# DiTEC-project/gnn-pressure-estimation

Hardware: AMD Instinct MI355X
Metric: train snapshots/sec (higher is better)
Workload: dtype f32; 1 GPU; gatres_small (15 blocks, nc=32), C-Town-sized WDN (388 nodes, 860 directed edges), batch_size=32 per GPU, fp32, full training step (device mask 0.95 -> fwd -> masked MSE -> bwd -> Adam), fused per-snapshot kernel (8 CUs per snapshot, row-window tables), hipGraph replay (20 steps per graph launch); global_batch=32, parallelism=dp1, plan_relabelled=False, row_window=92, dropped_steps=0, captured_graphs=25

## Files before the change

gnn-pressure-estimation_amd/csrc/gatres_layout.h:

```cpp
#pragma once
#include "gatres_common.h"

static inline __host__ __device__ int64_t r4(int64_t v) { return (v + 3) & ~(int64_t)3; }
#define GATRES_UREC_WORDS 128

struct Layout {
  int nb, nc;
  int64_t N, Eg;
  int64_t p_lin0_w, p_lin0_b, p_block0, p_block_stride, p_lin1_w, p_lin1_b, P;
  int64_t c1_as, c1_ad, c1_b, c1_W, c2_as, c2_ad, c2_b, c2_W;
  int64_t s_xin, s_h1, s_as1, s_ad1, s_al1, s_o1, s_h2, s_as2, s_ad2, s_al2, s_stride, saved_total;
  int64_t sc_y2, sc_ev, sc_xa, sc_xb, sc_gpa, sc_gpb, sc_gy2, sc_ge, sc_gad, sc_gas, sc_gh, sc_go1, sc_wt,
      sc_ge2, sc_gad2, sc_gas2, sc_gh2, sc_slabs, sc_loss_part, scratch_total;
  int64_t sc_px, sc_pmask, sc_pout, sc_pgout, sc_pgx;
  int64_t sc_wb;
  int64_t sc_xch, xch_stride;
  int64_t sc_urec;
  int64_t sc_keep, keep_stride, k_gh1, k_gh2, k_gas1, k_gad1, k_gas2, k_gad2;
  int split_max;
  int64_t sc_flags, flag_words, col_words, sc_part_slabs;
  int num_slabs;
  int slab_rows;
  int64_t slab_stride;
};
// ... 32 lines not shown
  int64_t o = 0;
  X.f1h = o; o += mn * 2 * nc;
  X.f1a = o; o += mn * 2;
  X.f2h = o; o += mn * nc;
  X.f2a = o; o += mn;
  X.f3 = o;  o += mn * nc;
  X.b1 = o;  o += mn * nc;
  X.b2y = o; o += mn * nc;
  X.b2e = o; o += me;
  X.b3o = o; o += mn * 2 * nc;
  X.b3e = o; o += me * 2;
  X.hb = o;  o += 6 * 8;
  X.total = (o + 15) & ~(int64_t)15;
  return X;
}

static inline bool make_layout(const gatres_model_t* m, int64_t N, int64_t Eg, int num_segments, int fused_nodes,
                               int fused_edges, Layout* L) {
  if (!m || m->num_blocks < 0 || N <= 0 || Eg < 0) return false;
  const int nc = m->nc, nb = m->num_blocks;
  if (nc < 4 || nc > 128 || !gatres_is_pow2(nc)) return false;
  L->nb = nb; L->nc = nc; L->N = N; L->Eg = Eg;
  const int64_t w = 2LL * nc * nc;
  L->p_lin0_w = 0; L->p_lin0_b = nc; L->p_block0 = 2LL * nc;
  L->c1_as = 0; L->c1_ad = 2LL * nc; L->c1_b = 4LL * nc; L->c1_W = 6LL * nc;
  L->c2_as = 6LL * nc + w; L->c2_ad = L->c2_as + nc; L->c2_b = L->c2_ad + nc; L->c2_W = L->c2_b + nc;
  L->p_block_stride = 9LL * nc + 2 * w;
  L->p_lin1_w = L->p_block0 + nb * L->p_block_stride;
  L->p_lin1_b = L->p_lin1_w + nc;
  L->P = L->p_lin1_b + 1;
// ... 62 lines not shown
    L->xch_stride = 2 * X.total;
    o += (int64_t)num_segments * L->xch_stride;
  }
  L->sc_urec = o;
  if (L->xch_stride > 0) o += (int64_t)((num_segments + 7) / 8) * 8 * 8 * GATRES_UREC_WORDS;
  L->sc_wb = o;    o += r4((int64_t)nb * 4 * nc * nc);
  L->sc_px = o;    o += r4(N);
  L->sc_pmask = o; o += r4((N + 3) / 4);
  L->sc_pout = o;  o += r4(N);
  L->sc_pgout = o; o += r4(N);
  L->sc_pgx = o;   o += r4(N);
  L->scratch_total = o;
  return true;
}

static inline int fused_nodes_of(const gatres_graph_t* g) {
  return (g && g->num_segments > 0 && g->seg_ptr && g->max_segment_nodes > 0 && g->max_segment_nodes <= 4096)
             ? g->max_segment_nodes : 0;
}
static inline bool make_layout_g(const gatres_model_t* m, const gatres_graph_t* g, Layout* L) {
  return g && make_layout(m, g->num_nodes, g->num_edges_gat, g->num_segments, fused_nodes_of(g),
                          g->max_segment_edges_gat, L);
}

constexpr int FUSED_STATUS_FAULT = 0, FUSED_STATUS_FAULT_COUNT = 1, FUSED_STATUS_FAULT_TICKETS = 2,
              FUSED_STATUS_DROPPED_STEPS = 3, FUSED_STATUS_SNAPSHOT = 8;
static inline int64_t fused_status_offset(const Layout& L) { return L.sc_flags + L.flag_words - 32; }
static inline unsigned* fused_status(float* scratch, const Layout& L) {
  return reinterpret_cast<unsigned*>(scratch + fused_status_offset(L));
}
// ... 28 lines not shown
```

gnn-pressure-estimation_amd/csrc/k_autoclip.hip:

```cpp
#include "gatres_common.h"
#include "k_autoclip.h"
#include "k_mask.h"
#include "k_update.h"

namespace {

constexpr int AC_NORM_MAX_BLOCKS = 256;
constexpr int AC_UPDATE_MAX_BLOCKS = 512;

__global__ __launch_bounds__(256) void autoclip_norm_kernel(const float* __restrict__ g, long long count, float grad_scale,
                                                            double* __restrict__ partials, unsigned long long* __restrict__ ctl,
                                                            const unsigned long long* __restrict__ step_counter, int drop_nan) {
  __shared__ double lds4[4];
  double s = 0.0;
  for (long long i = (long long)blockIdx.x * 256 + threadIdx.x; i < count; i += (long long)gridDim.x * 256) {
    const double x = (double)(g[i] * grad_scale);
    s += x * x;
  }
  s = ac_block_sum(s, lds4);
  if (threadIdx.x == 0) {
    partials[blockIdx.x] = s;
    if (blockIdx.x == 0) ac_snapshot(ctl, step_counter, drop_nan && g[0] != g[0]);
  }
}
// ... 94 lines not shown
  const long long gstride = (long long)a.update_blocks * 256;
  for (long long i = (long long)blockIdx.x * 256 + tid; i < t; i += gstride) B[i] = sorted_at(i);
  for (long long idx = (long long)blockIdx.x * 256 + tid; idx < a.u.count; idx += gstride) {
    const float pv = a.u.p[idx];
    float gv = a.u.g[idx] * a.u.grad_scale;
    gv = gv * coef;
    gv = gv + (float)wd * pv;
    float mv = a.u.m[idx];
    mv = mv + (float)(1.0 - b1) * (gv - mv);
    const float vv = (float)b2 * a.u.v[idx] + (float)(1.0 - b2) * gv * gv;
    const float denom = sqrtf(vv) / s_bc2_sqrt + (float)eps;
    const float pn = pv + (-s_step_size * mv) / denom;
    a.u.p[idx] = pn;
    a.u.m[idx] = mv;
    a.u.v[idx] = vv;
    if (a.u.wt) {
      const long long nc = a.u.nc, per = 2LL * nc * nc, stride = 9LL * nc + 2 * per, off = idx - 2LL * nc;
      if (off >= 0 && off < (long long)a.u.nb * stride) {
        const long long b = off / stride, o = off % stride;
        if (o >= 6LL * nc && o < 6LL * nc + per) {
          const long long e = o - 6LL * nc, row = e / nc, col = e % nc;
          a.u.wt[b * 2 * per + col * 2 * nc + row] = pn;
        } else if (o >= 9LL * nc + per) {
          const long long e = o - 9LL * nc - per, row = e / (2 * nc), col = e % (2 * nc);
          a.u.wt[b * 2 * per + per + col * nc + row] = pn;
        }
      }
    }
  }
}

bool ac_valid(const gatres_autoclip_t* ac) {
  return ac && ac->log && ac->sorted[0] && ac->sorted[1] && ac->sorted[0] != ac->sorted[1] && ac->ctl && ac->partials &&
         ac->norm_out && ac->clip_out && ac->coef_out && ac->capacity > 0 && ac->partials_cap > 0 &&
         ac->percentile >= 0.0 && ac->percentile <= 100.0;
}

}

extern "C" int32_t gatres_autoclip_partials(int64_t count) {
  return count <= 0 ? 0 : (int32_t)((count + 255) / 256);
}

// ... 47 lines not shown
```

gnn-pressure-estimation_amd/csrc/k_fused_host.hip:

```cpp
#include <atomic>
#include <vector>
#include "k_fused_dev.h"
#include "k_mask.h"
#include "k_autoclip.h"
#include "k_update.h"

namespace {

static unsigned long long* g_stamps = nullptr;
static int g_stamp_cap = 0;

struct SlabSumArgs {
  const float* slabs;
  int num_slabs, num_loss;
  long long stride;
  float* grads;
  const float* loss_part;
  float* loss;
  int do_adam, use_snap, reduce_blocks;
  unsigned* status;
  double* ac_partials;
  unsigned long long* ac_ctl;
};

// ... 64 lines not shown
    if constexpr (NORM) {
      const double x = (double)(acc * a.grad_scale);
      sq = fault ? 0.0 : x * x;
    }
    if (r.do_adam && !fault) {
      float gv = acc * a.grad_scale;
      gv = gv + (float)wd * pv;
      float mv = mv0;
      mv = mv + (float)(1.0 - b1) * (gv - mv);
      const float vv = (float)b2 * vv0 + (float)(1.0 - b2) * gv * gv;
      const float denom = sqrtf(vv) / s_bc2_sqrt + (float)eps;
      const float pn = pv + (-s_step_size * mv) / denom;
      a.p[idx] = pn;
      a.m[idx] = mv;
      a.v[idx] = vv;
      if (a.wt) {
        const long long per = 2LL * a.nc * a.nc, stride = 9LL * a.nc + 2 * per, off = idx - 2LL * a.nc;
        if (off >= 0 && off < (long long)a.nb * stride) {
          const long long b = off / stride, o = off % stride;
          if (o >= 6LL * a.nc && o < 6LL * a.nc + per) {
            const long long e = o - 6LL * a.nc, row = e / a.nc, col = e % a.nc;
            a.wt[b * 2 * per + col * 2 * a.nc + row] = pn;
          } else if (o >= 9LL * a.nc + per) {
            const long long e = o - 9LL * a.nc - per, row = e / (2 * a.nc), col = e % (2 * a.nc);
            a.wt[b * 2 * per + per + col * a.nc + row] = pn;
          }
        }
      }
    }
  }
  if constexpr (NORM) {
    __shared__ double lds4[4];
    sq = ac_block_sum(sq, lds4);
    if (threadIdx.x == 0) {
      r.ac_partials[blockIdx.x] = sq;
      if (blockIdx.x == 0) ac_snapshot(r.ac_ctl, a.step_counter, fault);
    }
  }
  if (fault && snap && blockIdx.x == 0 && threadIdx.x == 0) {
    r.status[FUSED_STATUS_FAULT_COUNT] += 1u;
    __hip_atomic_store(r.status, 0u, __ATOMIC_RELAXED, __HIP_MEMORY_SCOPE_AGENT);
  }
  if (fault && !snap && threadIdx.x == 0) {
// ... 75 lines not shown
    return make_float4(v.x, v.y, v.z, v.w);
  };
  auto update = [&](int64_t idx, float acc, float pv, float mv0, float vv0) {
    f.grads[idx] = fault ? NAN : acc;
    if (f.do_adam && !fault) {
      float gv = acc * f.u.grad_scale;
      gv = gv + (float)wd * pv;
      float mv = mv0;
      mv = mv + (float)(1.0 - b1) * (gv - mv);
      const float vv = (float)b2 * vv0 + (float)(1.0 - b2) * gv * gv;
      const float denom = sqrtf(vv) / s_bc2_sqrt + (float)eps;
      const float pn = pv + (-s_step_size * mv) / denom;
      f.u.p[idx] = pn;
      f.u.m[idx] = mv;
      f.u.v[idx] = vv;
      if (f.u.wt) {
        const long long per = 2LL * NC * NC, o = idx - po;
        if (o >= 6LL * NC && o < 6LL * NC + per) {
          const long long e = o - 6LL * NC, row = e / NC, cl = e % NC;
          f.u.wt[(long long)b * 2 * per + cl * 2 * NC + row] = pn;
        } else if (o >= 9LL * NC + per && o < 9LL * NC + 2 * per) {
          const long long e = o - 9LL * NC - per, row = e / (2 * NC), cl = e % (2 * NC);
          f.u.wt[(long long)b * 2 * per + per + cl * NC + row] = pn;
        }
      }
    }
  };
  auto finish_range = [&](int64_t lo, int64_t hi) {
    const int64_t n4 = (hi - lo) >> 2;
    for (int64_t q = tid; q < n4; q += PGR_THREADS) {
      const int64_t idx = lo + 4 * q;
      float4 pv = f4zero(), mv0 = f4zero(), vv0 = f4zero();
      if (f.do_adam && !fault) { pv = ld4(f.u.p + idx); mv0 = ld4(f.u.m + idx); vv0 = ld4(f.u.v + idx); }
      float4 acc = f4zero();
      int s0 = 0;
      for (; s0 + 12 <= S; s0 += 12) {
        float4 v12[12];
#pragma unroll
        for (int u = 0; u < 12; ++u) v12[u] = slab4(s0 + u, idx);
#pragma unroll
// ... 252 lines not shown
  out[GATRES_FUSED_PLAN_PARTS] = p.M;                 out[GATRES_FUSED_PLAN_WINDOW] = p.window;
  out[GATRES_FUSED_PLAN_CACHED] = p.cache;            out[GATRES_FUSED_PLAN_KEEP] = p.keep;
  out[GATRES_FUSED_PLAN_FACTS] = p.facts;             out[GATRES_FUSED_PLAN_LAUNCHES] = p.launches;
  out[GATRES_FUSED_PLAN_PER_LAUNCH] = p.per_launch;   out[GATRES_FUSED_PLAN_GRID] = p.grid0;
  out[GATRES_FUSED_PLAN_THREADS] = p.threads;         out[GATRES_FUSED_PLAN_PART_ROWS] = p.part_rows;
  out[GATRES_FUSED_PLAN_CUS] = p.cus;
  return rc;
}

extern "C" int gatres_fused_set_stamps(uint64_t* stamps, int32_t capacity) {
  g_stamps = reinterpret_cast<unsigned long long*>(stamps);
  g_stamp_cap = stamps ? capacity : 0;
  return 0;
}

extern "C" int gatres_fused_prepare_backward(const gatres_model_t* m, const gatres_graph_t* g, const float* params,
                                             float* scratch, void* stream) {
  if (!m || !g || !params || !scratch) return GATRES_E_BADARG;
  Layout L;
  if (!make_layout_g(m, g, &L)) return GATRES_E_UNSUPPORTED;
  return gatres_transpose_conv_weights(params, scratch + L.sc_wt, L.nb, L.nc, stream);
}

extern "C" int gatres_fused_run(const gatres_model_t* m, const gatres_graph_t* g, const float* params,
                                const float* x, const uint8_t* mask, const float* y, float* out, float* g_out,
                                float* loss_part, float* g_x, float* saved, float* scratch, int32_t phases,
                                void* stream) {
  if (!m || !g || !params || !x || !scratch) return GATRES_E_BADARG;
  if (!gatres_fused_supported(m, g)) return GATRES_E_UNSUPPORTED;
  FusedArgs a;
  if (!make_layout_g(m, g, &a.L)) return GATRES_E_UNSUPPORTED;
  if ((phases & GATRES_PHASE_FORWARD) && !out) return GATRES_E_BADARG;
  if ((phases & GATRES_PHASE_LOSS) && (!mask || !y || !out || !g_out || !loss_part)) return GATRES_E_BADARG;
  const int32_t crit_bits = phases & (GATRES_PHASE_LOSS_MAE | GATRES_PHASE_LOSS_SCE);
  if (crit_bits && (!(phases & GATRES_PHASE_LOSS) || crit_bits == (GATRES_PHASE_LOSS_MAE | GATRES_PHASE_LOSS_SCE)))
    return GATRES_E_BADARG;
// ... 133 lines not shown
  if ((loss_part == nullptr) != (loss == nullptr)) return GATRES_E_BADARG;
  if (!gatres_fused_supported(m, g)) return GATRES_E_UNSUPPORTED;
  ParamGradArgs a;
  if (!make_layout_g(m, g, &a.L)) return GATRES_E_UNSUPPORTED;
  if (!finish_folds(m, a.L)) return GATRES_E_UNSUPPORTED;
  if (block_lo < 0 || block_hi > a.L.nb || block_lo >= block_hi) return GATRES_E_BADARG;
  if (do_adam && (block_lo != 0 || block_hi != a.L.nb)) return GATRES_E_BADARG;
  a.seg_ptr = g->seg_ptr; a.saved = saved; a.keep = scratch + a.L.sc_keep; a.slabs = scratch + a.L.sc_slabs;
  a.M = fused_split(a.L, g); a.part_slabs = scratch + a.L.sc_part_slabs;
  a.SL = make_seg_layout(a.L.nb, a.L.nc, g->max_segment_nodes, g->max_segment_edges_gat);
  a.wt = scratch + a.L.sc_wt;
  FinishArgs f;
  f.u = update_args_of(params, nullptr, exp_avg, exp_avg_sq, step_counter, a.L.P, lr, beta1, beta2, eps, weight_decay, hparams,
                       grad_scale);
  f.u.wt = do_adam ? scratch + a.L.sc_wt : nullptr;
  f.grads = grads; f.loss_part = loss_part; f.loss = loss; f.num_loss = g->num_segments * a.M; f.do_adam = do_adam ? 1 : 0;
  f.status = fused_nodes_of(g) > 0 ? fused_status(scratch, a.L) : nullptr;
  f.colcnt = reinterpret_cast<unsigned*>(scratch + a.L.sc_flags + a.L.flag_words);
  f.S = g->num_segments; f.b_lo = block_lo; f.b_hi = block_hi; f.final_launch = block_lo == 0 ? 1 : 0;
  const dim3 grid((unsigned)(2 * (block_hi - block_lo) * g->num_segments));
  hipStream_t st = gatres_stream(stream);
  if (m->nc == 16) hipLaunchKernelGGL((param_grads_finish_kernel<16>), grid, dim3(PGR_THREADS), 0, st, a, f);
  else             hipLaunchKernelGGL((param_grads_finish_kernel<32>), grid, dim3(PGR_THREADS), 0, st, a, f);
  return gatres_launch_status();
}

extern "C" int gatres_fused_finish(const gatres_model_t* m, const gatres_graph_t* g, float* scratch, float* grads,
                                   const float* loss_part, float* loss, int32_t do_adam, float* params,
                                   float* exp_avg, float* exp_avg_sq, uint64_t* step_counter, double lr, double beta1,
                                   double beta2, double eps, double weight_decay, float grad_scale, void* stream) {
// ... 28 lines not shown
extern "C" __attribute__((visibility("hidden"))) int gatres_fused_finish_ex(
    const gatres_model_t* m, const gatres_graph_t* g, float* scratch, float* grads, const float* loss_part, float* loss,
    int32_t do_adam, const UpdateArgs& u, int32_t use_snap, void* stream) {
  if (!m || !g || !scratch || !grads) return GATRES_E_BADARG;
  if (u.mask_next && !use_snap) return GATRES_E_BADARG;
  if (u.mask_next && (!do_adam || !u.mask_node_ptr || u.mask_graphs <= 0 || !(u.mask_rate >= 0.0 && u.mask_rate <= 1.0)))
    return GATRES_E_BADARG;
  if (do_adam && (!u.p || !u.m || !u.v || !u.step_counter)) return GATRES_E_BADARG;
  if ((loss_part == nullptr) != (loss == nullptr)) return GATRES_E_BADARG;
  Layout L;
  SlabSumArgs r;
  if (!slab_sum_args(m, g, scratch, grads, loss_part, loss, &L, &r)) return GATRES_E_UNSUPPORTED;
  r.do_adam = do_adam; r.use_snap = (use_snap && do_adam) ? 1 : 0;
  UpdateArgs a = u;
  a.count = L.P;
  a.wt = do_adam ? scratch + L.sc_wt : nullptr; a.nb = L.nb; a.nc = L.nc;
  a.mask_snap = fused_status_snapshot(fused_status(scratch, L));
  const unsigned grid = (unsigned)(r.reduce_blocks + (a.mask_next ? a.mask_graphs * MASK_WGS_UPDATE : 0));
  hipLaunchKernelGGL(reduce_adam_kernel<false>, dim3(grid), dim3(256), 0, gatres_stream(stream), a, r);
  return gatres_launch_status();
}

extern "C" __attribute__((visibility("hidden"))) int gatres_fused_finish_norm_ex(
    const gatres_model_t* m, const gatres_graph_t* g, float* scratch, float* grads, const float* loss_part, float* loss,
    const UpdateArgs& u, const gatres_autoclip_t* ac, int32_t* num_partials, void* stream) {
  if (!m || !g || !scratch || !grads || !u.step_counter || !ac || !ac->partials || !ac->ctl || !num_partials) return GATRES_E_BADARG;
  if ((loss_part == nullptr) != (loss == nullptr)) return GATRES_E_BADARG;
  Layout L;
  SlabSumArgs r;
  if (!slab_sum_args(m, g, scratch, grads, loss_part, loss, &L, &r)) return GATRES_E_UNSUPPORTED;
  if (r.reduce_blocks > ac->partials_cap) return GATRES_E_BADARG;
// ... 8 lines not shown
```

gnn-pressure-estimation_amd/csrc/k_misc.hip:

```cpp
#include "gatres_common.h"
#include "k_conv_grads.h"
#include "k_mask.h"
#include "k_update.h"

#include <atomic>
#include <cstdlib>
#include <mutex>
namespace {
gatres_knobs_t g_knobs;
std::atomic<bool> g_knobs_ready{false};
std::mutex g_knobs_mu;
int env_flag(const char* n) { const char* e = getenv(n); return (e && *e && !(e[0] == '0' && !e[1])) ? 1 : 0; }
int env_int(const char* n, int dflt) { const char* e = getenv(n); return (e && *e) ? atoi(e) : dflt; }
void read_knobs(gatres_knobs_t* k) {
  k->fused_split = env_int("GATRES_FUSED_SPLIT", 0);
  k->fused_safe_sync = env_flag("GATRES_FUSED_SAFE_SYNC");
  k->fused_no_halo = env_flag("GATRES_FUSED_NO_HALO");
  k->fused_no_rounds = env_flag("GATRES_FUSED_NO_ROUNDS");
  const int lf = env_int("GATRES_AGG_LANE_FEATURES", 0);
  k->agg_lane_features = (lf == 4 || lf == 8) ? lf : 0;
  k->lin_bwd_wave = env_flag("GATRES_LIN_BWD_WAVE");
  k->no_proj_lds = env_flag("GATRES_NO_PROJ_LDS");
  k->dw_1d = env_flag("GATRES_DW_1D");
  k->side_stream = env_int("GATRES_SIDE_STREAM", -1);
// ... 473 lines not shown
  }
  __syncthreads();
  for (long long idx = (long long)blockIdx.x * 256 + threadIdx.x; idx < a.count; idx += (long long)update_blocks * 256) {
  {
    const float pv = a.p[idx];
    float gv = a.g[idx] * a.grad_scale;
    gv = gv + (float)wd * pv;
    float mv = a.m[idx];
    mv = mv + (float)(1.0 - b1) * (gv - mv);
    const float vv = (float)b2 * a.v[idx] + (float)(1.0 - b2) * gv * gv;
    const float denom = sqrtf(vv) / s_bc2_sqrt + (float)eps;
    const float pn = pv + (-s_step_size * mv) / denom;
    a.p[idx] = pn;
    a.m[idx] = mv;
    a.v[idx] = vv;
    if (a.wt) {
      const long long per = 2LL * a.nc * a.nc, stride = 9LL * a.nc + 2 * per, off = idx - 2LL * a.nc;
      if (off >= 0 && off < (long long)a.nb * stride) {
        const long long b = off / stride, o = off % stride;
        if (o >= 6LL * a.nc && o < 6LL * a.nc + per) {
          const long long e = o - 6LL * a.nc, row = e / a.nc, col = e % a.nc;
          a.wt[b * 2 * per + col * 2 * a.nc + row] = pn;
        } else if (o >= 9LL * a.nc + per) {
          const long long e = o - 9LL * a.nc - per, row = e / (2 * a.nc), col = e % (2 * a.nc);
          a.wt[b * 2 * per + per + col * a.nc + row] = pn;
        }
      }
    }
  }
  }
  if (!snap && threadIdx.x == 0 && done == (unsigned long long)update_blocks - 1ULL) {
    a.step_counter[1] = 0ULL;
    atomicAdd(&a.step_counter[0], 1ULL);
  }
}

}

#define GATRES_DISPATCH_T(dtype_, CALL_)                                  \
  switch (dtype_) {                                                       \
    case GATRES_DTYPE_F32: { using T = float; CALL_; break; }             \
    case GATRES_DTYPE_BF16: { using T = gatres_bf16; CALL_; break; }      \
    default: return GATRES_E_UNSUPPORTED;                                 \
// ... 228 lines not shown
```

gnn-pressure-estimation_amd/csrc/k_update.h:

```cpp
#pragma once
#include "gatres_common.h"

struct UpdateArgs {
  float* p;
  const float* g;
  float* m;
  float* v;
  unsigned long long* step_counter;
  long long count;
  double lr, b1, b2, eps, wd;
  const double* hp;
  float grad_scale;
  float* wt;
  int nb, nc;
  const int* mask_node_ptr;
  int mask_graphs;
  double mask_rate;
  unsigned long long mask_seed;
  uint8_t* mask_next;
  const unsigned long long* mask_snap;
  unsigned* drop_count;
};

static inline UpdateArgs update_args_of(float* params, const float* grads, float* exp_avg, float* exp_avg_sq,
                                        uint64_t* step_counter, int64_t count, double lr, double beta1, double beta2, double eps,
                                        double weight_decay, const double* hparams, float grad_scale) {
  UpdateArgs u{};
  u.p = params; u.g = grads; u.m = exp_avg; u.v = exp_avg_sq;
  u.step_counter = reinterpret_cast<unsigned long long*>(step_counter); u.count = count;
  u.lr = lr; u.b1 = beta1; u.b2 = beta2; u.eps = eps; u.wd = weight_decay; u.hp = hparams; u.grad_scale = grad_scale;
  return u;
}

extern "C" __attribute__((visibility("hidden"))) int gatres_adam_step_ex(const UpdateArgs& u, void* stream);

extern "C" __attribute__((visibility("hidden"))) int gatres_fused_finish_ex(
    const gatres_model_t* m, const gatres_graph_t* g, float* scratch, float* grads, const float* loss_part, float* loss,
// ... 10 lines not shown
```

gnn-pressure-estimation_amd/csrc/k_window.hip:

```cpp
#include <climits>
#include "k_window_stages.h"

namespace {

__device__ __forceinline__ void dma_land(int w0) {
  if ((int)__builtin_amdgcn_readfirstlane(threadIdx.x >> 6) >= w0) asm volatile("s_waitcnt vmcnt(0)" ::: "memory");
}
template <int THREADS>
__device__ __forceinline__ void vec_prefetch(float* dst, const float* __restrict__ src, int n) {
  const int lane = threadIdx.x & 63, wave = __builtin_amdgcn_readfirstlane(threadIdx.x >> 6);
  if (wave == THREADS / 64 - 1 && lane * 4 < n) __builtin_amdgcn_global_load_lds(src + lane * 4, dst, 16, 0, 0);
}
__device__ __forceinline__ int launder_s(int v) {
  asm volatile("" : "+s"(v));
  return v;
}

typedef const __attribute__((address_space(4))) FusedArgs* KArgs;
__device__ __forceinline__ KArgs kargs_fresh() {
  KArgs p = (KArgs)__builtin_amdgcn_kernarg_segment_ptr();
  asm volatile("" : "+s"(p));
  return p;
}
#define FRESH_ARGS()                                                                                          \
  const KArgs ka_ = kargs_fresh();                                                                            \
  [[maybe_unused]] const auto& L = ka_->L; [[maybe_unused]] const auto& SL = ka_->SL; [[maybe_unused]] const auto& XL = ka_->XL
// ... 45 lines not shown
    float* p = gpT + (size_t)r * NC + idx % NC;
    *p = *p / cnt;
  }
}

template <int NC, int THREADS, int PH = -1>
__global__ __launch_bounds__(THREADS) void gatres_window_kernel(const FusedArgs a) {
  const int ph_ = PH < 0 ? a.phases : (PH & 0xff);
  const bool keep_ = PH < 0 ? a.keep_lds != 0 : (PH & 0x100) != 0;
  constexpr bool SYM = PH >= 0 && (PH & 0x200) != 0;
  constexpr bool NOHUB = PH >= 0 && (PH & 0x400) != 0;
  constexpr bool PTAB = PH >= 0 && (PH & 0x800) != 0;
  constexpr bool OW64 = PH >= 0 && (PH & 0x1000) != 0;
  constexpr bool HOIST = NC == 32 && THREADS == 1024 && NOHUB && PTAB && OW64;
  constexpr bool SWEEP = HOIST && !(PH & 0x8000);
  constexpr bool NOSAVE = PH >= 0 && (PH & 0x2000) != 0 && (PH & 0xff) == GATRES_PHASE_FORWARD;
  constexpr bool XLOCAL = PH >= 0 && (PH & 0x4000) != 0;
  const bool mse_ = PH < 0 ? a.criterion == GATRES_LOSS_MSE : (PH & 0x8000) == 0;
#ifdef GATRES_NO_XPAD
  constexpr int XPF = 0, XPB = 0;
#else
  constexpr int XPF = (NC == 32 && NOHUB) ? 4 : 0;
  constexpr int XPB = (NC == 32 && PH >= 0 && (PH & 0x100) != 0) ? 4 : 0;
#endif
  __shared__ __attribute__((aligned(16))) unsigned char lds_raw[LDS_BYTES];
  float* ldsf = reinterpret_cast<float*>(lds_raw);
  const Layout& L = a.L;
  const int M = a.M;
  const int within = blockIdx.x % (8 * M);
  const int seg = a.seg0 + (blockIdx.x / (8 * M)) * 8 + (within & 7), part = within >> 3;
// ... 48 lines not shown
  xc.base_hb = xc.base + XL.hb;
  xc.M = M; xc.part = part; xc.err = a.err; xc.local = grp.local;
  xc.dead = GATRES_DIAG && (a.no_halo & 2) != 0;
  xc.ep = (unsigned)uni((int)__hip_atomic_load(grp.flags + part * FLAG_STRIDE + 2, __ATOMIC_RELAXED, __HIP_MEMORY_SCOPE_AGENT));
  const XchBuf xbuf = xch_buffer(xc.base, XL.total);
  const bool pace = SYM ? false : !a.sym;
  constexpr int PW = 8;
  const int dw0 = NC == 32 ? PW : min((ow + 15) >> 4, THREADS / 64 - 4);
  constexpr int WL_FLOATS = 2 * NC * (2 * NC + 4) + 4 * NC;
  constexpr int WLB = (WL_FLOATS + 3) & ~3;
  constexpr int B1OFF = 2 * NC * (NC + 4) + 4 * NC;
  constexpr int B2OFF = NC * (2 * NC + 4) + 2 * NC;
  constexpr int A2OFF = 2 * NC * (NC + 4);
  constexpr int A1OFF = NC * (2 * NC + 4);
  static_assert(B1OFF + 2 * NC <= WLB && B2OFF + NC <= WLB && A2OFF + 2 * NC <= WLB && A1OFF + 4 * NC <= WLB, "W slot tails");
  const float* P = a.params;
  float* sc = a.scratch;
  unsigned char* lds_top = lds_raw + LDS_BYTES - (keep_ ? win_keep_bytes(L.nb, ow) : 0);
  unsigned long long* mo1 = keep_ ? reinterpret_cast<unsigned long long*>(lds_top) - lo : nullptr;
  unsigned* mxin = keep_ ? reinterpret_cast<unsigned*>(lds_top + 8LL * L.nb * ow) - lo : nullptr;
  [[maybe_unused]] int stamp_i = 0;
  STAMP();
  if (STAMPS_PTR && blockIdx.x == 0 && threadIdx.x == 0) STAMPS_PTR[a.stamp_cap] = clock64();

  int wlo, whi, elo, oeg, ewlo, weg, melo, oem, tlo, otg, mtlo, otm;
  if (PTAB || pt) {
    wlo = H(GATRES_PT_WLO); whi = H(GATRES_PT_WHI); elo = H(GATRES_PT_ELO); oeg = H(GATRES_PT_OEG); ewlo = H(GATRES_PT_EWLO);
    weg = H(GATRES_PT_WEG); melo = H(GATRES_PT_MELO); oem = H(GATRES_PT_OEM); tlo = H(GATRES_PT_TLO); otg = H(GATRES_PT_OTG);
    mtlo = H(GATRES_PT_MTLO); otm = H(GATRES_PT_OTM);
  } else {
// ... 353 lines not shown
        float* xnext = segbase + (int64_t)(launder_s(b) + 1) * SL.bstride + SL.xin;
        win_mean_fwd<NC, THREADS, NOHUB, NC + XPF, HOIST>(rw, mbin, mrp, mcolo, y2T, xA, NOSAVE ? nullptr : xnext, xA,
                                       (mxin && b + 1 < nb) ? mxin + (b + 1) * ow : nullptr, qm2);
        lds_barrier();
        STAMP();
      }
    }
    if (assume_local && !(ph_ & GATRES_PHASE_BACKWARD)) group_verify_local(grp);
#ifndef GATRES_NO_L2_TOUCH
    if constexpr (PTAB && NC == 32) {
      if (ph_ & GATRES_PHASE_BACKWARD) {
        const int b0 = H(GATRES_PT_B_IMG);
        for (int k = b0 + tid * 32; k < a.ptab_stride; k += THREADS * 32) (void)*reinterpret_cast<const volatile int*>(pt + k);
        if (L.nb > 0 && tid >= THREADS / 2) {
          const int t2 = tid - THREADS / 2;
          constexpr int WT_LINES = 2 * NC * NC / 32;
          const float* wt2 = a.wt + (int64_t)(L.nb - 1) * 4 * NC * NC + 2 * NC * NC;
          if (t2 < WT_LINES) (void)*reinterpret_cast<const volatile float*>(wt2 + t2 * 32);
          else if (t2 < WT_LINES + 2)
            (void)*reinterpret_cast<const volatile float*>(P + L.p_block0 + (int64_t)(L.nb - 1) * L.p_block_stride + L.c2_as + (t2 - WT_LINES) * 32);
        }
      }
    }
#endif
    FRESH_FWD();
#define LIST_(T_, N_, I_) I_(lo) I_(hi) T_(float, xA)
    REC_LOADS(LIST_);
    REC_DEFS(LIST_);
#undef LIST_
    {
      constexpr int G = NC / 4;
      const float4 wv = ld4(P + L.p_lin1_w + (tid % G) * 4);
      const float bias = P[L.p_lin1_b];
      const int rounds = (rw.hi - rw.lo + THREADS / G - 1) / (THREADS / G);
      float cnt = 0.f;
// ... 193 lines not shown
    float* ge2 = gew - ewlo;      float* ge1 = gew - ewlo * 2;
    float* gad2 = gado - lo;      float* gad1 = gado - lo * 2;
    float* hT2 = hTw - wlo * NC;  float* hT1 = hTw - wlo * 2 * NC;
    float* asT2 = asTw - wlo;     float* asT1 = asTw - wlo * 2;
    float* adT2 = adTo - lo;      float* adT1 = adTo - lo * 2;
    float* alT2 = alTw - ewlo;    float* alT1 = alTw - ewlo * 2;
    float* xG2 = xGo - lo * (NC + XPB);   float* xG1 = xGo - lo * (2 * NC + XPB);
    float* gkeep = keep_ ? gko - lo * NC : nullptr;

    const float* xfinal = segbase + (int64_t)L.nb * SL.bstride + SL.xin;
    auto dma_conv2_early = [&](int blk, int w0) {
      if (wave_u < w0) return;
      FRESH_ARGS();
      blk = launder_s(blk);
      const float* bs = segbase + (int64_t)blk * SL.bstride;
      dma_copy16<THREADS>(hTw, bs + SL.h2 + (size_t)wlo * NC, wr * NC, w0);
      dma_copy4<THREADS>(asTw, bs + SL.as2 + wlo, wr, w0);
      dma_copy4<THREADS>(adTo, bs + SL.ad2 + lo, ow, w0);
      w_prefetch<NC, 2 * NC, EPI_RESID_MASK, THREADS>(wlA, a.wt + (int64_t)blk * 2 * w + w, nullptr, nullptr, w0);
      vec_prefetch<THREADS>(wlA + A2OFF, P + L.p_block0 + (int64_t)blk * L.p_block_stride + L.c2_as, 2 * NC);
    };
    auto dma_conv2_late = [&](int blk, int w0) {
      if (wave_u < w0) return;
      FRESH_ARGS();
      blk = launder_s(blk);
      const float* bs = segbase + (int64_t)blk * SL.bstride;
      dma_copy4<THREADS>(alTw, bs + SL.al2 + ewlo, weg, w0);
    };
    if (L.nb > 0) { dma_conv2_early(L.nb - 1, 0); dma_conv2_late(L.nb - 1, 0); }
    if (fuse_loss) {
      const int c = tid % NC, rg = tid / NC;
      const float wv = P[L.p_lin1_w + c];
      float aw = 0.f, ab = 0.f;
#pragma unroll
      for (int k = 0; k < 2; ++k) {
// ... 75 lines not shown
    auto xout = [&](bool on, const unsigned char* bflag, unsigned t_rows, unsigned t_small) {
      XOut o;
      o.xb = xbuf; o.ep = xc.ep + 1u; o.local = xc.local; o.on = on; o.flag = bflag; o.t_rows = t_rows; o.t_small = t_small;
      return o;
    };
    auto dma_conv2_early = [&](int blk, int w0) {
      if (wave_u < w0) return;
      FRESH_ARGS(); FRESH_BWD();
#define LIST_(T_, N_, I_) I_(lo) I_(hi) T_(float, hTw) T_(float, asTw) T_(float, adTo) T_(float, wlA) I_(wlo) I_(wr) I_(ow)
      REC_LOADS(LIST_);
      REC_PINS(LIST_);
      REC_DEFS(LIST_);
#undef LIST_
      blk = launder_s(blk);
      const float* bs = segbase + (int64_t)blk * SL.bstride;
      dma_copy16<THREADS>(hTw, bs + SL.h2 + (size_t)wlo * NC, wr * NC, w0);
      dma_copy4<THREADS>(asTw, bs + SL.as2 + wlo, wr, w0);
      dma_copy4<THREADS>(adTo, bs + SL.ad2 + lo, ow, w0);
      w_prefetch<NC, 2 * NC, EPI_RESID_MASK, THREADS>(wlA, a.wt + (int64_t)blk * 2 * w + w, nullptr, nullptr, w0);
      vec_prefetch<THREADS>(wlA + A2OFF, P + L.p_block0 + (int64_t)blk * L.p_block_stride + L.c2_as, 2 * NC);
    };
    auto dma_conv2_late = [&](int blk, int w0) {
      if (wave_u < w0) return;
      FRESH_ARGS(); FRESH_BWD();
#define LIST_(T_, N_, I_) I_(lo) I_(hi) T_(float, alTw) I_(ewlo) I_(weg)
      REC_LOADS(LIST_);
      REC_PINS(LIST_);
      REC_DEFS(LIST_);
#undef LIST_
      blk = launder_s(blk);
      const float* bs = segbase + (int64_t)blk * SL.bstride;
      dma_copy4<THREADS>(alTw, bs + SL.al2 + ewlo, weg, w0);
    };
    [[maybe_unused]] uint4 bn1 = uint4{}, bn2 = uint4{}, bma = uint4{}, bmb = uint4{}, bt1a = uint4{}, bt1b = uint4{};
    if constexpr (HOIST) {
// ... 329 lines not shown
```

gnn-pressure-estimation_amd/csrc/train_driver.hip:

```cpp
#include "gatres_common.h"
#include "gatres_layout.h"
#include "k_update.h"

static bool wants_mask_next(const gatres_train_step_t* ts) {
  return (ts->flags & GATRES_FLAG_MASK_NEXT) && ts->node_ptr && ts->num_graphs > 0 && ts->mask_next && ts->mask_next != ts->mask;
}

static UpdateArgs update_args(const gatres_train_step_t* ts, float* wt, uint32_t* drop_count, bool sample_ahead) {
  UpdateArgs u = update_args_of(ts->params, ts->grads, ts->exp_avg, ts->exp_avg_sq, ts->step_counter,
                                gatres_param_count(ts->model.num_blocks, ts->model.nc), ts->lr, ts->beta1, ts->beta2, ts->eps,
                                ts->weight_decay, ts->hparams, ts->grad_scale);
  if (wt) { u.wt = wt; u.nb = ts->model.num_blocks; u.nc = ts->model.nc; }
  u.drop_count = drop_count;
  if (sample_ahead) {
    u.mask_node_ptr = ts->node_ptr; u.mask_graphs = ts->num_graphs; u.mask_rate = ts->mask_rate; u.mask_seed = ts->seed;
    u.mask_next = ts->mask_next;
  }
  return u;
}

static int autoclip_update(const gatres_train_step_t* ts, const UpdateArgs& u, void* stream) {
  int32_t np = 0;
  const int rc = gatres_autoclip_norm_ex(u, ts->autoclip, &np, stream);
  return rc ? rc : gatres_autoclip_update_ex(u, ts->autoclip, np, stream);
}

static int fused_grads_and_update(const gatres_train_step_t* ts, float* wt, const float* loss_part, bool adam, void* stream) {
  const bool snap_later = !adam && (ts->flags & GATRES_FLAG_MASK_NEXT) && ts->step_counter;
  const int rc = gatres_fused_param_grads_ex(&ts->model, ts->graph, ts->saved, ts->scratch,
                                             (adam || snap_later) ? ts->step_counter : nullptr, stream);
  if (rc < 0 || rc > 1) return rc;
  const UpdateArgs u = update_args(ts, wt, nullptr, adam && wants_mask_next(ts) && rc == 1);
  float* loss = loss_part ? ts->loss : nullptr;
  if (adam && ts->autoclip) {
    int32_t np = 0;
    const int rc2 = gatres_fused_finish_norm_ex(&ts->model, ts->graph, ts->scratch, ts->grads, loss_part, loss, u, ts->autoclip,
                                                &np, stream);
    return rc2 ? rc2 : gatres_autoclip_update_ex(u, ts->autoclip, np, stream);
  }
  return gatres_fused_finish_ex(&ts->model, ts->graph, ts->scratch, ts->grads, loss_part, loss, adam ? 1 : 0, u,
                                rc == 1 ? 1 : 0, stream);
}

extern "C" int gatres_train_step(const gatres_train_step_t* ts, void* stream) {
  if (!ts || !ts->graph || !ts->params || !ts->x || !ts->y || !ts->mask || !ts->out || !ts->g_out || !ts->loss ||
      !ts->saved || !ts->scratch)
    return GATRES_E_BADARG;
// ... 14 lines not shown
    if (!ac->log || !ac->sorted[0] || !ac->sorted[1] || !ac->ctl || !ac->partials || !ac->norm_out || !ac->clip_out ||
        !ac->coef_out || ac->capacity <= 0 || ac->partials_cap < gatres_autoclip_partials(gatres_param_count(ts->model.num_blocks, ts->model.nc)) ||
        !(ac->percentile >= 0.0 && ac->percentile <= 100.0))
      return GATRES_E_BADARG;
  }
  if ((ts->phases & GATRES_PHASE_MASK) && ts->node_ptr) {
    rc = gatres_mask_generate(ts->node_ptr, ts->num_graphs, ts->mask_rate, ts->seed, ts->step_counter, ts->mask,
                              stream);
    if (rc) return rc;
  }
  if (fused) {
    Layout L;
    if (!make_layout_g(&ts->model, ts->graph, &L)) return GATRES_E_UNSUPPORTED;
    float* loss_part = ts->scratch + L.sc_loss_part;
    float* wt = ts->scratch + L.sc_wt;
    const bool fwd = ts->phases & GATRES_PHASE_FORWARD, bwd = ts->phases & GATRES_PHASE_BACKWARD;
    const bool adam = ts->phases & GATRES_PHASE_ADAM;
    if ((bwd && !ts->grads) || (adam && (!ts->grads || !ts->exp_avg || !ts->exp_avg_sq || !ts->step_counter)))
      return GATRES_E_BADARG;
    const bool deferred = (ts->flags & GATRES_FLAG_GRADS_DEFERRED) != 0;
    if (ts->flags & GATRES_FLAG_GRADS_ONLY) {
      if (!bwd || fwd || adam) return GATRES_E_BADARG;
      const bool top = ts->block_hi == ts->model.num_blocks;
      return gatres_fused_param_grads_finish(&ts->model, ts->graph, ts->saved, ts->scratch, ts->grads,
                                             top ? loss_part : nullptr, top ? ts->loss : nullptr, 0, nullptr, nullptr,
                                             nullptr, nullptr, 0., 0., 0., 0., 0., nullptr, 1.f, ts->block_lo, ts->block_hi,
                                             stream);
    }
    if (bwd && !(ts->flags & GATRES_FLAG_WT_VALID)) {
      rc = gatres_fused_prepare_backward(&ts->model, ts->graph, ts->params, ts->scratch, stream);
      if (rc) return rc;
    }
    if (fwd && bwd) {
      rc = gatres_fused_run(&ts->model, ts->graph, ts->params, ts->x, ts->mask, ts->y, ts->out, ts->g_out, loss_part,
                            nullptr, ts->saved, ts->scratch,
                            GATRES_PHASE_FORWARD | loss_phase | GATRES_PHASE_BACKWARD, stream);
      if (rc || deferred) return rc;
      return fused_grads_and_update(ts, wt, loss_part, adam, stream);
    }
    if (fwd) {
      rc = gatres_fused_run(&ts->model, ts->graph, ts->params, ts->x, ts->mask, nullptr, ts->out, nullptr, nullptr,
                            nullptr, ts->saved, ts->scratch, GATRES_PHASE_FORWARD, stream);
      if (rc) return rc;
      rc = gatres_masked_loss(ts->out, ts->y, ts->mask, crit, ts->loss, ts->g_out, N, stream);
      if (rc) return rc;
    }
    if (bwd) {
      rc = gatres_fused_run(&ts->model, ts->graph, ts->params, ts->x, ts->mask, nullptr, nullptr, ts->g_out, nullptr,
                            nullptr, ts->saved, ts->scratch, GATRES_PHASE_BACKWARD, stream);
      if (rc || deferred) return rc;
      return fused_grads_and_update(ts, wt, nullptr, adam, stream);
    }
    if (adam) {
      uint32_t* status = fused_status(ts->scratch, L);
      const bool next = wants_mask_next(ts);
      if (next && !gatres_fused_finish_folds(&ts->model, ts->graph)) return GATRES_E_UNSUPPORTED;
      UpdateArgs u = update_args(ts, wt, status + FUSED_STATUS_DROPPED_STEPS, next);
      u.mask_snap = fused_status_snapshot(status);
      return ts->autoclip ? autoclip_update(ts, u, stream) : gatres_adam_step_ex(u, stream);
    }
    return 0;
  }
  if (ts->phases & GATRES_PHASE_FORWARD) {
    rc = gatres_model_forward_per_op(&ts->model, ts->graph, ts->params, ts->x, ts->mask, ts->out, ts->saved, ts->scratch,
                              stream);
    if (rc) return rc;
    rc = gatres_masked_loss(ts->out, ts->y, ts->mask, crit, ts->loss, ts->g_out, N, stream);
    if (rc) return rc;
  }
  if (ts->phases & GATRES_PHASE_BACKWARD) {
    if (!ts->grads) return GATRES_E_BADARG;
    rc = gatres_model_backward_per_op(&ts->model, ts->graph, ts->params, ts->x, ts->mask, ts->g_out, ts->saved, ts->scratch,
                               ts->grads, nullptr, stream);
    if (rc) return rc;
  }
  if (ts->phases & GATRES_PHASE_ADAM) {
    if (!ts->grads || !ts->exp_avg || !ts->exp_avg_sq || !ts->step_counter) return GATRES_E_BADARG;
    const UpdateArgs u = update_args(ts, nullptr, nullptr, false);
    return ts->autoclip ? autoclip_update(ts, u, stream) : gatres_adam_step_ex(u, stream);
  }
  return 0;
}
```

Baseline: 108,800 snapshots/s.

## Store conv2 weights as padded LDS slot image for single DMA copy

Adds a per-block weight image in scratch (at sc_wb) laid out exactly like the LDS W slot (transposed conv2 W padded to nc+4 columns plus attention vectors). Adam and the prepare kernel now write this image alongside the transposed copy. The fused backward kernel then loads the slot with one linear global_load_lds copy instead of a strided w_prefetch plus a separate vector prefetch. This aims to cut LDS staging instructions and latency in the conv2 backward DMA, at the cost of extra scattered stores in the optimizer and more scratch use.

```diff
diff --git a/gnn-pressure-estimation_amd/csrc/gatres_layout.h b/gnn-pressure-estimation_amd/csrc/gatres_layout.h
--- a/gnn-pressure-estimation_amd/csrc/gatres_layout.h
+++ b/gnn-pressure-estimation_amd/csrc/gatres_layout.h
@@ -70,6 +70,9 @@
   X.total = (o + 15) & ~(int64_t)15;
   return X;
 }
+
+static constexpr __host__ __device__ int64_t wimg2_floats(int nc) { return 2LL * nc * (nc + 4) + 2 * nc; }
+static constexpr __host__ __device__ int64_t wimg_block_floats(int nc) { return nc == 32 ? wimg2_floats(nc) : 0; }
 
 static inline bool make_layout(const gatres_model_t* m, int64_t N, int64_t Eg, int num_segments, int fused_nodes,
                                int fused_edges, Layout* L) {
@@ -162,6 +165,8 @@
   return true;
 }
 
+static inline float* wimg_of(float* scratch, const Layout& L) { return wimg_block_floats(L.nc) > 0 ? scratch + L.sc_wb : nullptr; }
+
 static inline int fused_nodes_of(const gatres_graph_t* g) {
   return (g && g->num_segments > 0 && g->seg_ptr && g->max_segment_nodes > 0 && g->max_segment_nodes <= 4096)
              ? g->max_segment_nodes : 0;
diff --git a/gnn-pressure-estimation_amd/csrc/k_autoclip.hip b/gnn-pressure-estimation_amd/csrc/k_autoclip.hip
--- a/gnn-pressure-estimation_amd/csrc/k_autoclip.hip
+++ b/gnn-pressure-estimation_amd/csrc/k_autoclip.hip
@@ -132,19 +132,7 @@
     a.u.p[idx] = pn;
     a.u.m[idx] = mv;
     a.u.v[idx] = vv;
-    if (a.u.wt) {
-      const long long nc = a.u.nc, per = 2LL * nc * nc, stride = 9LL * nc + 2 * per, off = idx - 2LL * nc;
-      if (off >= 0 && off < (long long)a.u.nb * stride) {
-        const long long b = off / stride, o = off % stride;
-        if (o >= 6LL * nc && o < 6LL * nc + per) {
-          const long long e = o - 6LL * nc, row = e / nc, col = e % nc;
-          a.u.wt[b * 2 * per + col * 2 * nc + row] = pn;
-        } else if (o >= 9LL * nc + per) {
-          const long long e = o - 9LL * nc - per, row = e / (2 * nc), col = e % (2 * nc);
-          a.u.wt[b * 2 * per + per + col * nc + row] = pn;
-        }
-      }
-    }
+    if (a.u.wt) conv_copies_store_flat(a.u.wt, a.u.wimg, a.u.nb, a.u.nc, idx, pn);
   }
 }
 
diff --git a/gnn-pressure-estimation_amd/csrc/k_fused_host.hip b/gnn-pressure-estimation_amd/csrc/k_fused_host.hip
--- a/gnn-pressure-estimation_amd/csrc/k_fused_host.hip
+++ b/gnn-pressure-estimation_amd/csrc/k_fused_host.hip
@@ -102,19 +102,7 @@
       a.p[idx] = pn;
       a.m[idx] = mv;
       a.v[idx] = vv;
-      if (a.wt) {
-        const long long per = 2LL * a.nc * a.nc, stride = 9LL * a.nc + 2 * per, off = idx - 2LL * a.nc;
-        if (off >= 0 && off < (long long)a.nb * stride) {
-          const long long b = off / stride, o = off % stride;
-          if (o >= 6LL * a.nc && o < 6LL * a.nc + per) {
-            const long long e = o - 6LL * a.nc, row = e / a.nc, col = e % a.nc;
-            a.wt[b * 2 * per + col * 2 * a.nc + row] = pn;
-          } else if (o >= 9LL * a.nc + per) {
-            const long long e = o - 9LL * a.nc - per, row = e / (2 * a.nc), col = e % (2 * a.nc);
-            a.wt[b * 2 * per + per + col * a.nc + row] = pn;
-          }
-        }
-      }
+      if (a.wt) conv_copies_store_flat(a.wt, a.wimg, a.nb, a.nc, idx, pn);
     }
   }
   if constexpr (NORM) {
@@ -220,16 +208,7 @@
       f.u.p[idx] = pn;
       f.u.m[idx] = mv;
       f.u.v[idx] = vv;
-      if (f.u.wt) {
-        const long long per = 2LL * NC * NC, o = idx - po;
-        if (o >= 6LL * NC && o < 6LL * NC + per) {
-          const long long e = o - 6LL * NC, row = e / NC, cl = e % NC;
-          f.u.wt[(long long)b * 2 * per + cl * 2 * NC + row] = pn;
-        } else if (o >= 9LL * NC + per && o < 9LL * NC + 2 * per) {
-          const long long e = o - 9LL * NC - per, row = e / (2 * NC), cl = e % (2 * NC);
-          f.u.wt[(long long)b * 2 * per + per + cl * NC + row] = pn;
-        }
-      }
+      if (f.u.wt) conv_copies_store(f.u.wt, f.u.wimg, NC, b, idx - po, pn);
     }
   };
   auto finish_range = [&](int64_t lo, int64_t hi) {
@@ -512,12 +491,24 @@
   return 0;
 }
 
+__global__ __launch_bounds__(256) void conv_copies_kernel(const float* __restrict__ params, float* wt, float* wimg, int nb, int nc) {
+  const long long stride = 9LL * nc + 4LL * nc * nc, idx = (long long)blockIdx.x * 256 + threadIdx.x;
+  if (idx >= (long long)nb * stride) return;
+  const long long b = idx / stride, o = idx % stride;
+  conv_copies_store(wt, wimg, nc, b, o, params[2LL * nc + idx]);
+  if (wimg && o < 4LL * 2 * nc) wimg[b * wimg_block_floats(nc) + (o >> 2) * (nc + 4) + nc + (o & 3)] = 0.f;
+}
+
 extern "C" int gatres_fused_prepare_backward(const gatres_model_t* m, const gatres_graph_t* g, const float* params,
                                              float* scratch, void* stream) {
   if (!m || !g || !params || !scratch) return GATRES_E_BADARG;
   Layout L;
   if (!make_layout_g(m, g, &L)) return GATRES_E_UNSUPPORTED;
-  return gatres_transpose_conv_weights(params, scratch + L.sc_wt, L.nb, L.nc, stream);
+  if (L.nb == 0) return 0;
+  const long long count = (long long)L.nb * L.p_block_stride;
+  hipLaunchKernelGGL(conv_copies_kernel, dim3((unsigned)((count + 255) / 256)), dim3(256), 0, gatres_stream(stream), params,
+                     scratch + L.sc_wt, wimg_of(scratch, L), L.nb, L.nc);
+  return gatres_launch_status();
 }
 
 extern "C" int gatres_fused_run(const gatres_model_t* m, const gatres_graph_t* g, const float* params,
@@ -681,6 +672,7 @@
   f.u = update_args_of(params, nullptr, exp_avg, exp_avg_sq, step_counter, a.L.P, lr, beta1, beta2, eps, weight_decay, hparams,
                        grad_scale);
   f.u.wt = do_adam ? scratch + a.L.sc_wt : nullptr;
+  f.u.wimg = do_adam ? wimg_of(scratch, a.L) : nullptr;
   f.grads = grads; f.loss_part = loss_part; f.loss = loss; f.num_loss = g->num_segments * a.M; f.do_adam = do_adam ? 1 : 0;
   f.status = fused_nodes_of(g) > 0 ? fused_status(scratch, a.L) : nullptr;
   f.colcnt = reinterpret_cast<unsigned*>(scratch + a.L.sc_flags + a.L.flag_words);
@@ -739,7 +731,7 @@
   r.do_adam = do_adam; r.use_snap = (use_snap && do_adam) ? 1 : 0;
   UpdateArgs a = u;
   a.count = L.P;
-  a.wt = do_adam ? scratch + L.sc_wt : nullptr; a.nb = L.nb; a.nc = L.nc;
+  a.wt = do_adam ? scratch + L.sc_wt : nullptr; a.wimg = do_adam ? wimg_of(scratch, L) : nullptr; a.nb = L.nb; a.nc = L.nc;
   a.mask_snap = fused_status_snapshot(fused_status(scratch, L));
   const unsigned grid = (unsigned)(r.reduce_blocks + (a.mask_next ? a.mask_graphs * MASK_WGS_UPDATE : 0));
   hipLaunchKernelGGL(reduce_adam_kernel<false>, dim3(grid), dim3(256), 0, gatres_stream(stream), a, r);
diff --git a/gnn-pressure-estimation_amd/csrc/k_misc.hip b/gnn-pressure-estimation_amd/csrc/k_misc.hip
--- a/gnn-pressure-estimation_amd/csrc/k_misc.hip
+++ b/gnn-pressure-estimation_amd/csrc/k_misc.hip
@@ -511,19 +511,7 @@
     a.p[idx] = pn;
     a.m[idx] = mv;
     a.v[idx] = vv;
-    if (a.wt) {
-      const long long per = 2LL * a.nc * a.nc, stride = 9LL * a.nc + 2 * per, off = idx - 2LL * a.nc;
-      if (off >= 0 && off < (long long)a.nb * stride) {
-        const long long b = off / stride, o = off % stride;
-        if (o >= 6LL * a.nc && o < 6LL * a.nc + per) {
-          const long long e = o - 6LL * a.nc, row = e / a.nc, col = e % a.nc;
-          a.wt[b * 2 * per + col * 2 * a.nc + row] = pn;
-        } else if (o >= 9LL * a.nc + per) {
-          const long long e = o - 9LL * a.nc - per, row = e / (2 * a.nc), col = e % (2 * a.nc);
-          a.wt[b * 2 * per + per + col * a.nc + row] = pn;
-        }
-      }
-    }
+    if (a.wt) conv_copies_store_flat(a.wt, a.wimg, a.nb, a.nc, idx, pn);
   }
   }
   if (!snap && threadIdx.x == 0 && done == (unsigned long long)update_blocks - 1ULL) {
diff --git a/gnn-pressure-estimation_amd/csrc/k_update.h b/gnn-pressure-estimation_amd/csrc/k_update.h
--- a/gnn-pressure-estimation_amd/csrc/k_update.h
+++ b/gnn-pressure-estimation_amd/csrc/k_update.h
@@ -1,5 +1,6 @@
 #pragma once
 #include "gatres_common.h"
+#include "gatres_layout.h"
 
 struct UpdateArgs {
   float* p;
@@ -12,6 +13,7 @@
   const double* hp;
   float grad_scale;
   float* wt;
+  float* wimg;
   int nb, nc;
   const int* mask_node_ptr;
   int mask_graphs;
@@ -21,6 +23,24 @@
   const unsigned long long* mask_snap;
   unsigned* drop_count;
 };
+
+__device__ __forceinline__ void conv_copies_store(float* wt, float* wimg, long long nc, long long b, long long o, float v) {
+  const long long per = 2 * nc * nc;
+  if (o >= 6 * nc && o < 6 * nc + per) {
+    const long long e = o - 6 * nc, row = e / nc, col = e % nc;
+    wt[b * 2 * per + col * 2 * nc + row] = v;
+  } else if (o >= 9 * nc + per && o < 9 * nc + 2 * per) {
+    const long long e = o - 9 * nc - per, row = e / (2 * nc), col = e % (2 * nc);
+    wt[b * 2 * per + per + col * nc + row] = v;
+    if (wimg) wimg[b * wimg_block_floats((int)nc) + col * (nc + 4) + row] = v;
+  } else if (wimg && o >= 6 * nc + per && o < 8 * nc + per) {
+    wimg[b * wimg_block_floats((int)nc) + 2 * nc * (nc + 4) + (o - 6 * nc - per)] = v;
+  }
+}
+__device__ __forceinline__ void conv_copies_store_flat(float* wt, float* wimg, long long nb, long long nc, long long idx, float v) {
+  const long long stride = 9 * nc + 4 * nc * nc, off = idx - 2 * nc;
+  if (off >= 0 && off < nb * stride) conv_copies_store(wt, wimg, nc, off / stride, off % stride, v);
+}
 
 static inline UpdateArgs update_args_of(float* params, const float* grads, float* exp_avg, float* exp_avg_sq,
                                         uint64_t* step_counter, int64_t count, double lr, double beta1, double beta2, double eps,
diff --git a/gnn-pressure-estimation_amd/csrc/k_window.hip b/gnn-pressure-estimation_amd/csrc/k_window.hip
--- a/gnn-pressure-estimation_amd/csrc/k_window.hip
+++ b/gnn-pressure-estimation_amd/csrc/k_window.hip
@@ -10,6 +10,15 @@
 __device__ __forceinline__ void vec_prefetch(float* dst, const float* __restrict__ src, int n) {
   const int lane = threadIdx.x & 63, wave = __builtin_amdgcn_readfirstlane(threadIdx.x >> 6);
   if (wave == THREADS / 64 - 1 && lane * 4 < n) __builtin_amdgcn_global_load_lds(src + lane * 4, dst, 16, 0, 0);
+}
+template <int THREADS, int N>
+__device__ __forceinline__ void dma_copy16_n(float* dst, const float* src, int w0) {
+  const int lane = threadIdx.x & 63, wave = __builtin_amdgcn_readfirstlane(threadIdx.x >> 6);
+  if (wave < w0) return;
+  const int nw = THREADS / 64 - w0;
+#pragma unroll
+  for (int k = 0; k < (N + 255) / 256; ++k)
+    if (k % nw == wave - w0 && k * 256 + lane * 4 < N) __builtin_amdgcn_global_load_lds(src + k * 256 + lane * 4, dst + k * 256, 16, 0, 0);
 }
 __device__ __forceinline__ int launder_s(int v) {
   asm volatile("" : "+s"(v));
@@ -85,6 +94,13 @@
   constexpr bool OW64 = PH >= 0 && (PH & 0x1000) != 0;
   constexpr bool HOIST = NC == 32 && THREADS == 1024 && NOHUB && PTAB && OW64;
   constexpr bool SWEEP = HOIST && !(PH & 0x8000);
+#ifdef GATRES_NO_WIMG
+  constexpr bool IMG = false;
+#else
+  constexpr bool IMG = HOIST && !(PH & 0x8000);
+#endif
+  constexpr int IMG2 = 2 * NC * (NC + 4) + 2 * NC;
+  [[maybe_unused]] constexpr int IMGS = IMG ? (int)wimg_block_floats(NC) : 0;
   constexpr bool NOSAVE = PH >= 0 && (PH & 0x2000) != 0 && (PH & 0xff) == GATRES_PHASE_FORWARD;
   constexpr bool XLOCAL = PH >= 0 && (PH & 0x4000) != 0;
   const bool mse_ = PH < 0 ? a.criterion == GATRES_LOSS_MSE : (PH & 0x8000) == 0;
@@ -163,6 +179,7 @@
   constexpr int A2OFF = 2 * NC * (NC + 4);
   constexpr int A1OFF = NC * (2 * NC + 4);
   static_assert(B1OFF + 2 * NC <= WLB && B2OFF + NC <= WLB && A2OFF + 2 * NC <= WLB && A1OFF + 4 * NC <= WLB, "W slot tails");
+  static_assert(IMG2 == A2OFF + 2 * NC && IMG2 % 4 == 0 && (!IMG || (IMGS >= IMG2 && IMGS % 4 == 0)), "slot image");
   const float* P = a.params;
   float* sc = a.scratch;
   unsigned char* lds_top = lds_raw + LDS_BYTES - (keep_ ? win_keep_bytes(L.nb, ow) : 0);
@@ -546,11 +563,16 @@
         for (int k = b0 + tid * 32; k < a.ptab_stride; k += THREADS * 32) (void)*reinterpret_cast<const volatile int*>(pt + k);
         if (L.nb > 0 && tid >= THREADS / 2) {
           const int t2 = tid - THREADS / 2;
+          if constexpr (IMG) {
+            const float* img = a.scratch + L.sc_wb + (int64_t)(L.nb - 1) * IMGS;
+            for (int k = t2 * 32; k < IMG2; k += THREADS / 2 * 32) (void)*reinterpret_cast<const volatile float*>(img + k);
+          } else {
           constexpr int WT_LINES = 2 * NC * NC / 32;
           const float* wt2 = a.wt + (int64_t)(L.nb - 1) * 4 * NC * NC + 2 * NC * NC;
           if (t2 < WT_LINES) (void)*reinterpret_cast<const volatile float*>(wt2 + t2 * 32);
           else if (t2 < WT_LINES + 2)
             (void)*reinterpret_cast<const volatile float*>(P + L.p_block0 + (int64_t)(L.nb - 1) * L.p_block_stride + L.c2_as + (t2 - WT_LINES) * 32);
+          }
         }
       }
     }
@@ -774,11 +796,14 @@
       FRESH_ARGS();
       blk = launder_s(blk);
       const float* bs = segbase + (int64_t)blk * SL.bstride;
+      if constexpr (IMG) dma_copy16_n<THREADS, IMG2>(wlA, a.scratch + L.sc_wb + (int64_t)blk * IMGS, w0);
       dma_copy16<THREADS>(hTw, bs + SL.h2 + (size_t)wlo * NC, wr * NC, w0);
       dma_copy4<THREADS>(asTw, bs + SL.as2 + wlo, wr, w0);
       dma_copy4<THREADS>(adTo, bs + SL.ad2 + lo, ow, w0);
-      w_prefetch<NC, 2 * NC, EPI_RESID_MASK, THREADS>(wlA, a.wt + (int64_t)blk * 2 * w + w, nullptr, nullptr, w0);
-      vec_prefetch<THREADS>(wlA + A2OFF, P + L.p_block0 + (int64_t)blk * L.p_block_stride + L.c2_as, 2 * NC);
+      if constexpr (!IMG) {
+        w_prefetch<NC, 2 * NC, EPI_RESID_MASK, THREADS>(wlA, a.wt + (int64_t)blk * 2 * w + w, nullptr, nullptr, w0);
+        vec_prefetch<THREADS>(wlA + A2OFF, P + L.p_block0 + (int64_t)blk * L.p_block_stride + L.c2_as, 2 * NC);
+      }
     };
     auto dma_conv2_late = [&](int blk, int w0) {
       if (wave_u < w0) return;
@@ -884,11 +909,14 @@
 #undef LIST_
       blk = launder_s(blk);
       const float* bs = segbase + (int64_t)blk * SL.bstride;
+      if constexpr (IMG) dma_copy16_n<THREADS, IMG2>(wlA, a.scratch + L.sc_wb + (int64_t)blk * IMGS, w0);
       dma_copy16<THREADS>(hTw, bs + SL.h2 + (size_t)wlo * NC, wr * NC, w0);
       dma_copy4<THREADS>(asTw, bs + SL.as2 + wlo, wr, w0);
       dma_copy4<THREADS>(adTo, bs + SL.ad2 + lo, ow, w0);
-      w_prefetch<NC, 2 * NC, EPI_RESID_MASK, THREADS>(wlA, a.wt + (int64_t)blk * 2 * w + w, nullptr, nullptr, w0);
-      vec_prefetch<THREADS>(wlA + A2OFF, P + L.p_block0 + (int64_t)blk * L.p_block_stride + L.c2_as, 2 * NC);
+      if constexpr (!IMG) {
+        w_prefetch<NC, 2 * NC, EPI_RESID_MASK, THREADS>(wlA, a.wt + (int64_t)blk * 2 * w + w, nullptr, nullptr, w0);
+        vec_prefetch<THREADS>(wlA + A2OFF, P + L.p_block0 + (int64_t)blk * L.p_block_stride + L.c2_as, 2 * NC);
+      }
     };
     auto dma_conv2_late = [&](int blk, int w0) {
       if (wave_u < w0) return;
diff --git a/gnn-pressure-estimation_amd/csrc/train_driver.hip b/gnn-pressure-estimation_amd/csrc/train_driver.hip
--- a/gnn-pressure-estimation_amd/csrc/train_driver.hip
+++ b/gnn-pressure-estimation_amd/csrc/train_driver.hip
@@ -6,11 +6,11 @@
   return (ts->flags & GATRES_FLAG_MASK_NEXT) && ts->node_ptr && ts->num_graphs > 0 && ts->mask_next && ts->mask_next != ts->mask;
 }
 
-static UpdateArgs update_args(const gatres_train_step_t* ts, float* wt, uint32_t* drop_count, bool sample_ahead) {
+static UpdateArgs update_args(const gatres_train_step_t* ts, float* wt, float* wimg, uint32_t* drop_count, bool sample_ahead) {
   UpdateArgs u = update_args_of(ts->params, ts->grads, ts->exp_avg, ts->exp_avg_sq, ts->step_counter,
                                 gatres_param_count(ts->model.num_blocks, ts->model.nc), ts->lr, ts->beta1, ts->beta2, ts->eps,
                                 ts->weight_decay, ts->hparams, ts->grad_scale);
-  if (wt) { u.wt = wt; u.nb = ts->model.num_blocks; u.nc = ts->model.nc; }
+  if (wt) { u.wt = wt; u.wimg = wimg; u.nb = ts->model.num_blocks; u.nc = ts->model.nc; }
   u.drop_count = drop_count;
   if (sample_ahead) {
     u.mask_node_ptr = ts->node_ptr; u.mask_graphs = ts->num_graphs; u.mask_rate = ts->mask_rate; u.mask_seed = ts->seed;
@@ -25,12 +25,13 @@
   return rc ? rc : gatres_autoclip_update_ex(u, ts->autoclip, np, stream);
 }
 
-static int fused_grads_and_update(const gatres_train_step_t* ts, float* wt, const float* loss_part, bool adam, void* stream) {
+static int fused_grads_and_update(const gatres_train_step_t* ts, float* wt, float* wimg, const float* loss_part, bool adam,
+                                  void* stream) {
   const bool snap_later = !adam && (ts->flags & GATRES_FLAG_MASK_NEXT) && ts->step_counter;
   const int rc = gatres_fused_param_grads_ex(&ts->model, ts->graph, ts->saved, ts->scratch,
                                              (adam || snap_later) ? ts->step_counter : nullptr, stream);
   if (rc < 0 || rc > 1) return rc;
-  const UpdateArgs u = update_args(ts, wt, nullptr, adam && wants_mask_next(ts) && rc == 1);
+  const UpdateArgs u = update_args(ts, wt, wimg, nullptr, adam && wants_mask_next(ts) && rc == 1);
   float* loss = loss_part ? ts->loss : nullptr;
   if (adam && ts->autoclip) {
     int32_t np = 0;
@@ -75,6 +76,7 @@
     if (!make_layout_g(&ts->model, ts->graph, &L)) return GATRES_E_UNSUPPORTED;
     float* loss_part = ts->scratch + L.sc_loss_part;
     float* wt = ts->scratch + L.sc_wt;
+    float* wimg = wimg_of(ts->scratch, L);
     const bool fwd = ts->phases & GATRES_PHASE_FORWARD, bwd = ts->phases & GATRES_PHASE_BACKWARD;
     const bool adam = ts->phases & GATRES_PHASE_ADAM;
     if ((bwd && !ts->grads) || (adam && (!ts->grads || !ts->exp_avg || !ts->exp_avg_sq || !ts->step_counter)))
@@ -97,7 +99,7 @@
                             nullptr, ts->saved, ts->scratch,
                             GATRES_PHASE_FORWARD | loss_phase | GATRES_PHASE_BACKWARD, stream);
       if (rc || deferred) return rc;
-      return fused_grads_and_update(ts, wt, loss_part, adam, stream);
+      return fused_grads_and_update(ts, wt, wimg, loss_part, adam, stream);
     }
     if (fwd) {
       rc = gatres_fused_run(&ts->model, ts->graph, ts->params, ts->x, ts->mask, nullptr, ts->out, nullptr, nullptr,
@@ -110,13 +112,13 @@
       rc = gatres_fused_run(&ts->model, ts->graph, ts->params, ts->x, ts->mask, nullptr, nullptr, ts->g_out, nullptr,
                             nullptr, ts->saved, ts->scratch, GATRES_PHASE_BACKWARD, stream);
       if (rc || deferred) return rc;
-      return fused_grads_and_update(ts, wt, nullptr, adam, stream);
+      return fused_grads_and_update(ts, wt, wimg, nullptr, adam, stream);
     }
     if (adam) {
       uint32_t* status = fused_status(ts->scratch, L);
       const bool next = wants_mask_next(ts);
       if (next && !gatres_fused_finish_folds(&ts->model, ts->graph)) return GATRES_E_UNSUPPORTED;
-      UpdateArgs u = update_args(ts, wt, status + FUSED_STATUS_DROPPED_STEPS, next);
+      UpdateArgs u = update_args(ts, wt, wimg, status + FUSED_STATUS_DROPPED_STEPS, next);
       u.mask_snap = fused_status_snapshot(status);
       return ts->autoclip ? autoclip_update(ts, u, stream) : gatres_adam_step_ex(u, stream);
     }
@@ -137,7 +139,7 @@
   }
   if (ts->phases & GATRES_PHASE_ADAM) {
     if (!ts->grads || !ts->exp_avg || !ts->exp_avg_sq || !ts->step_counter) return GATRES_E_BADARG;
-    const UpdateArgs u = update_args(ts, nullptr, nullptr, false);
+    const UpdateArgs u = update_args(ts, nullptr, nullptr, nullptr, false);
     return ts->autoclip ? autoclip_update(ts, u, stream) : gatres_adam_step_ex(u, stream);
   }
   return 0;
```

Result: no change. 109,200 snapshots/s (median of 2 runs) (+0.4%).
